# salute-developers/GigaAM

Hardware: AMD Instinct MI355X
Metric: RTFx v2_ctc batch32x20s (log-mel + encoder + greedy decode) (higher is better)
Workload: dtype f32 (GEMMs: 3-term split on fp16 MFMA, fp32 accumulate)

## Files before the change

gigaam_amd/_lib.py:

```python
from __future__ import annotations

import ctypes as C
import os
from typing import Optional

_HERE = os.path.dirname(os.path.abspath(__file__))
LIB_NAME = "libgigaam_hip.so"
LIB_PATH = os.path.join(_HERE, LIB_NAME)

SUBS_CONV2D, SUBS_CONV1D = 0, 1
ATT_ROTARY, ATT_REL_POS = 0, 1
NORM_BATCH, NORM_LAYER = 0, 1
HEAD_NONE, HEAD_CTC, HEAD_RNNT, HEAD_EMO = 0, 1, 2, 3
DTYPE_F32, DTYPE_F16, DTYPE_BF16, DTYPE_F64, DTYPE_I64 = 0, 1, 2, 3, 4
GEMM_F32, GEMM_F16X3, GEMM_F16 = 0, 1, 2
RS_U8, RS_I16, RS_I24, RS_I32, RS_F32, RS_MULAW, RS_ALAW = range(7)
RS_FORM_SINGLE, RS_FORM_TABLE, RS_FORM_ROWS = 0, 1, 2
PF_CLASSES = ["gemm", "conv2", "attn", "norm", "convmod", "stem", "frontend", "decode", "misc", "align_bt", "align_out"]


class GamConfig(C.Structure):
    _fields_ = [(n, C.c_int32) for n in (
        "sample_rate", "n_mels", "hop_length", "win_length", "n_fft", "center",
        "feat_in", "n_layers", "d_model", "subsampling", "subs_kernel_size", "subsampling_factor",
# ... 61 lines not shown
    "gam_rnnt_align": (C.c_int, [_P, _P, _P, C.c_int, C.c_int64, _P, _P, C.c_int, _P, _P, _P, _P, _P]),
    "gam_op_rnnt_align": (C.c_int, [_P, _P, _P, C.c_int, C.c_int64, _P, _P, C.c_int, _P, _P, _P, _P, _P, _P]),
    "gam_op_rnnt_lattice_align": (C.c_int, [_P, _P, _P, C.c_int, C.c_int64, C.c_int, _P, _P, C.c_int, _P, _P, _P, _P, _P]),
    "gam_set_rnnt_align_workspace": (C.c_int, [_P, C.c_int64]),
    "gam_ctc_confidence": (C.c_int, [_P, _P, _P, C.c_int, C.c_int64, _P, _P, _P, C.c_int, C.c_int, C.c_int, _P, _P, _P, _P]),
    "gam_op_ctc_confidence": (C.c_int, [_P, _P, _P, C.c_int, C.c_int64, C.c_int, _P, _P, _P, C.c_int, C.c_int, C.c_int, _P, _P, _P, _P]),
    "gam_op_ctc_confidence_long": (C.c_int, [_P, _P, C.c_int64, C.c_int, _P, _P, _P, C.c_int, C.c_int, C.c_int, C.c_int, _P, _P, _P, _P]),
    "gam_rnnt_confidence": (C.c_int, [_P, _P, _P, C.c_int, C.c_int64, _P, _P, _P, C.c_int, C.c_int, _P, _P, _P]),
    "gam_op_rnnt_confidence": (C.c_int, [_P, _P, _P, C.c_int, C.c_int64, _P, _P, _P, C.c_int, C.c_int, _P, _P, _P]),
    "gam_emo_probs": (C.c_int, [_P, _P, _P, C.c_int, C.c_int64, _P, _P]),
    "gam_rnnt_predict": (C.c_int, [_P, _P, _P, _P, C.c_int, _P, _P, _P, _P]),
    "gam_rnnt_joint": (C.c_int, [_P, _P, _P, C.c_int, C.c_int, C.c_int, _P, _P]),
    "gam_set_gemm_mode": (C.c_int, [_P, C.c_int]),
    "gam_get_gemm_mode": (C.c_int, [_P]),
    "gam_set_rnnt_cluster": (C.c_int, [_P, C.c_int]),
    "gam_get_rnnt_cluster": (C.c_int, [_P]),
    "gam_rnnt_cluster_plan_info": (C.c_int, [C.c_int] * 8 + [C.POINTER(C.c_int32)]),
    "gam_rnnt_last_decode": (C.c_int, [_P, C.POINTER(C.c_int32)]),
    "gam_debug_buffer_hash": (C.c_int, [_P, C.c_int, C.POINTER(C.c_uint64), C.POINTER(C.c_int64)]),
    "gam_range_flag": (C.c_int, [_P, C.POINTER(C.c_int), _P]),
    "gam_range_flag_fetch": (C.c_int, [_P, _P, _P]),
    "gam_op_gemm": (C.c_int, [_P, _P, _P, _P, _P, C.c_int, C.c_int, C.c_int, C.c_int, _P]),
    "gam_op_gemm_ex": (C.c_int, [_P, _P, _P, _P, _P, C.c_float, _P, C.c_int, C.c_int, C.c_int, C.c_int, _P]),
    "gam_op_attention": (C.c_int, [_P, _P, _P, _P, _P, _P, C.c_int, C.c_int, C.c_int, _P]),
    "gam_op_attention_ex": (C.c_int, [_P, _P, _P, _P, C.c_int64, _P, _P, _P, C.c_int, C.c_int, C.c_int, C.c_int, _P, _P, _P, _P]),
    "gam_op_layernorm": (C.c_int, [_P, C.POINTER(GamLnOp), _P]),
    "gam_op_convmod": (C.c_int, [_P, _P, _P, _P, _P, _P, _P, _P, _P, C.c_int, C.c_int, C.c_int, C.c_int, C.c_int, C.c_int, C.c_int, _P]),
    "gam_tune_sp": (C.c_int, [C.c_int, C.c_int, C.c_int]),
    "gam_plan_sp": (C.c_int, [C.c_int, C.c_int, C.c_int, C.c_int, C.POINTER(C.c_int), C.POINTER(C.c_int), C.POINTER(C.c_int)]),
    "gam_plan_sp_ex": (C.c_int, [C.c_int, C.c_int, C.c_int, C.c_int, C.POINTER(C.c_int), C.POINTER(C.c_int), C.POINTER(C.c_int), C.POINTER(C.c_int)]),
    "gam_tune_sp_stages": (C.c_int, [C.c_int]),
    "gam_resample_plan": (C.c_int, [C.c_int, C.c_int, C.POINTER(C.c_int), C.POINTER(C.c_int), C.POINTER(C.c_int)]),
    "gam_resample_tile": (C.c_int, [C.c_int, C.c_int, C.POINTER(C.c_int), C.POINTER(C.c_int)]),
    "gam_resample_table": (C.c_int, [C.c_int, C.c_int, _P, _P]),
    "gam_resample_out_len": (C.c_int64, [C.c_int, C.c_int, C.c_int64]),
    "gam_op_resample": (C.c_int, [_P, C.c_int, C.c_int, C.c_int, _P, C.c_int, C.c_int64, C.c_int, C.c_int, _P, _P, _P, C.c_int64, _P, _P]),
    "gam_profile_enable": (C.c_int, [_P, C.c_int]),
    "gam_profile_pause": (C.c_int, [_P, C.c_int]),
    "gam_profile_read": (C.c_int, [_P, C.c_int, C.POINTER(C.c_double), C.POINTER(C.c_int64), C.POINTER(C.c_double)]),
    "gam_profile_read_bytes": (C.c_int, [_P, C.c_int, C.POINTER(C.c_double)]),
    "gam_last_error": (C.c_char_p, [_P]),
    "gam_comm_unique_id": (C.c_int, [C.c_char_p]),
    "gam_comm_create": (C.c_int, [C.c_char_p, C.c_int, C.c_int, C.c_int, C.POINTER(_P)]),
    "gam_comm_world": (C.c_int, [_P]),
    "gam_gather_ids": (C.c_int, [_P, _P, _P, _P, _P, C.c_int, C.c_int, _P, _P, _P, _P, _P]),
    "gam_comm_last_error": (C.c_char_p, [_P]),
# ... 30 lines not shown
```

gigaam_amd/csrc/gam_api.hip:

```cpp
#include <hip/hip_runtime.h>

#include <algorithm>
#include <cmath>
#include <cstdarg>
#include <cstdio>
#include <cstring>
#include <map>
#include <string>
#include <vector>

#include "../../include/gigaam_hip.h"
#include "gam_align.h"
#include "gam_align_long.h"
#include "gam_kws.h"
#include "gam_attn.h"
#include "gam_beam.h"
#include "gam_beam_stream.h"
#include "gam_rnnt_beam.h"
#include "gam_attn16.h"
#include "gam_comm.h"
#include "gam_common.h"
#include "gam_convmod.h"
#include "gam_decode.h"
#include "gam_rnnt_align.h"
// ... 2621 lines not shown
  HIPCHK(h, hipGetLastError());
  return 0;
}

int gam_emo_probs(gam_handle* h, const float* encoded, const int32_t* enc_len, int B, int64_t Tp, float* probs,
                  void* stream) {
  if (int r = head_check(h, GAM_HEAD_EMO, nullptr)) return r;
  if (B <= 0 || Tp <= 0 || !encoded || !probs) return fail(h, -1, "bad emotion-head arguments");
  HIPCHK(h, hipSetDevice(h->device));
  hipStream_t s = (hipStream_t)stream;
  const int D = h->cfg.d_model, NC = h->cfg.num_classes;
  ProfScope ps(h, s, GAM_PF_DECODE, (double)B * D * Tp * 4.0);
  hipLaunchKernelGGL(gam_emo_head_kernel, dim3(B), dim3(256), (size_t)(D + NC) * sizeof(float), s, encoded, enc_len,
                     h->emo_w, h->emo_b, probs, D, (int)Tp, NC);
  HIPCHK(h, hipGetLastError());
  return 0;
}

int gam_op_gemm(gam_handle* h, const float* A, const float* W, const float* bias, float* C, int M, int N, int K, int act,
                void* stream) {
  return gam_op_gemm_ex(h, A, W, bias, nullptr, 1.0f, C, M, N, K, act, stream);
}

int gam_op_gemm_ex(gam_handle* h, const float* A, const float* W, const float* bias, const float* R, float alpha, float* C, int M,
                   int N, int K, int act, void* stream) {
  if (!h) return -1;
  HIPCHK(h, hipSetDevice(h->device));
  GamGemmArgs g = gemm_args(A, K, W, bias, C, N, M, N, K);
  g.R = R; g.ldr = N; g.alpha = alpha;
  hipStream_t s = (hipStream_t)stream;
  if (!split_mode(h) || K % 32 != 0 || N % 4 != 0) return gemm(h, s, g, act);
  const size_t wn = (size_t)N * K, an = (size_t)M * K;
  W16 w16;
  if (int r = ensure(h, h->op_sp, wn + 64)) return r;
  hipLaunchKernelGGL(gam_to_sp32_kernel, dim3((int)std::min<size_t>((wn / 4 + 255) / 256, 4096)), dim3(256), 0, s, W,
                     (_Float16*)h->op_sp.p, wn / 4, (const float*)nullptr, K);
  w16.sp = (_Float16*)h->op_sp.p;
  if (int r = ensure(h, h->op_rs, (size_t)M + 64)) return r;
  hipLaunchKernelGGL(gam_rowscale_kernel, dim3(gam_cdiv(M, 4)), dim3(256), 0, s, A, h->op_rs.p, M, K, (long)K);
  g.a_rs = h->op_rs.p;
  if (int r = ensure(h, h->aplanes, an + 64)) return r;
  g.Asp = (const _Float16*)h->aplanes.p;
  g.a_fmt = (h->gemm_mode == GAM_GEMM_F16 && K % 64 == 0) ? 2 : 1;
  if (g.a_fmt == 2) {
    if (int r = ensure(h, h->op_planes, wn / 2 + 64)) return r;
    w16.h16 = (_Float16*)h->op_planes.p;
    hipLaunchKernelGGL(gam_to_h16_kernel, dim3((int)std::min<size_t>((wn / 4 + 255) / 256, 4096)), dim3(256), 0, s, W, w16.h16,
                       wn / 4, (const float*)nullptr, K);
    hipLaunchKernelGGL(gam_to_h16_kernel, dim3((int)std::min<size_t>((an / 4 + 255) / 256, 8192)), dim3(256), 0, s, A,
                       (_Float16*)h->aplanes.p, an / 4, (const float*)h->op_rs.p, K);
  } else {
    hipLaunchKernelGGL(gam_to_sp32_kernel, dim3((int)std::min<size_t>((an / 4 + 255) / 256, 8192)), dim3(256), 0, s, A,
// ... 264 lines not shown
```

gigaam_amd/csrc/gam_gemm_sp.h:

```cpp
#pragma once
#include "gam_gemm.h"
#include <type_traits>
#if defined(GAM_SP_INSTRUMENT) && GAM_SP_INSTRUMENT
#include <algorithm>
#include <vector>
#endif

#ifndef GAM_SP_INSTRUMENT
#define GAM_SP_INSTRUMENT 0
#endif
#if GAM_SP_INSTRUMENT
#define GAM_SP_TL(i)                                                                  \
  if (g.tlog != nullptr && threadIdx.x == 0) {                                        \
    g.tlog[(size_t)lid * 8 + (i)] = wall_clock64();                                   \
    if ((i) == 1 || (i) == 2) g.tlog[(size_t)lid * 8 + 4 + (i)] = clock64();          \
    if ((i) == 0) g.tlog[(size_t)lid * 8 + 7] = blockIdx.x;                            \
  }
#else
#define GAM_SP_TL(i)
#endif

template <int MT, int NW, int NS = 2>
struct GamGemmSpCfg {
  static constexpr int BM = 64 * MT;
  static constexpr int BN = 64 * NW;
  static constexpr int NWAVES = 2 * NW;
  static constexpr int NT = 64 * NWAVES;
  static constexpr int A_BYTES = BM * 128;
  static constexpr int W_BYTES = BN * 128;
  static constexpr int STAGE = A_BYTES + W_BYTES;
  static constexpr int SMEM = NS * STAGE;
  static constexpr int NAI = BM / 8 / NWAVES;
  static constexpr int NWI = BN / 8 / NWAVES;
};

__device__ __forceinline__ int gam_sp_key(int row) { return ((row >> 1) & 7) ^ ((row >> 3) & 2); }

template <int ACT, int MT, int NW, int NS = 2, bool H16 = false>
__global__ __launch_bounds__(128 * NW, NW == 2 ? 2 : 1) void gam_gemm_sp_kernel(GamGemmArgs g) {
  extern __shared__ __attribute__((aligned(16))) unsigned char gam_smem_sp[];
  using Cfg = GamGemmSpCfg<MT, NW, NS>;
  constexpr int BM = Cfg::BM, BN = Cfg::BN, NAI = Cfg::NAI, NWI = Cfg::NWI, NWAVES = Cfg::NWAVES;
  typedef __attribute__((address_space(3))) void* lds_ptr_t;
  typedef const __attribute__((address_space(1))) void* glb_ptr_t;

  const int tid = threadIdx.x;
  const int lane = tid & 63;
  const int wave = __builtin_amdgcn_readfirstlane(tid >> 6);
  const int wm = wave / NW, wn = wave % NW;

  const int nbn = (g.N + BN - 1) / BN;
  const int total = gridDim.x;
  const int q8 = total >> 3, r8 = total & 7;
  const int bid = blockIdx.x;
  const int xcd = bid & 7;
  const int lid = (xcd < r8 ? xcd * (q8 + 1) : r8 * (q8 + 1) + (xcd - r8) * q8) + (bid >> 3);
  int tm = lid / nbn, tn = lid % nbn;
  if (g.skip_pad) {
    tm = bid / nbn;
    tn = bid % nbn;
  }
// ... 171 lines not shown
  for (int kt = 0; kt < nk; ++kt) {
    const int s_nxt = s_cur + 1 == NS ? 0 : s_cur + 1;
    const unsigned char* st = gam_smem_sp + s_cur * Cfg::STAGE;
    const unsigned char* sn = gam_smem_sp + s_nxt * Cfg::STAGE;
    half0(st);
    if constexpr (NS == 2) {
      __builtin_amdgcn_s_waitcnt(0x0070);
      __syncthreads();
    } else {
      asm volatile("s_waitcnt vmcnt(%0) lgkmcnt(0)\n\ts_barrier" ::"n"(VMW) : "memory");
    }
    half1(sn, s_cur);
    s_cur = s_nxt;
  }
#undef GAM_SPLD
#undef GAM_SP_RDW
#undef GAM_SP_RDA
#undef GAM_SP_MFMA
  __builtin_amdgcn_s_waitcnt(0x0070);
  GAM_SP_TL(2);

  const int mw = m0 + wm * (BM / 2), nw = n0 + wn * 64;

  const int lrow = lane & 15, lq8 = (lane >> 4) * 8;
  const float accscale = g.wscale_inv;
  f32x4 bv[2][2];
#pragma unroll
  for (int pp = 0; pp < 2; ++pp)
#pragma unroll
    for (int hf = 0; hf < 2; ++hf) {
      const int col = nw + 32 * pp + lq8 + 4 * hf;
      bv[pp][hf] = (g.bias != nullptr && col < g.N) ? *reinterpret_cast<const f32x4*>(g.bias + col) : (f32x4){0.f, 0.f, 0.f, 0.f};
    }
  const bool part = g.partial != nullptr;
  const bool need_bt = !part && (g.lens != nullptr || g.remap);
  bool r_ok[2 * MT], r_masked[2 * MT];
  long r_orow[2 * MT];
  float r_rsc[2 * MT];
  int bb = 0, tt = 0;
  if (need_bt) { bb = (mw + lrow) / g.rpb; tt = (mw + lrow) - bb * g.rpb; }
#pragma unroll
  for (int i = 0; i < 2 * MT; ++i) {
    const int row = mw + 16 * i + lrow;
    bool ok = row < g.M, masked = false;
    long orow = row;
    if (need_bt) {
      if (i > 0) {
        tt += 16;
        if (g.rpb < 16) { bb = row / g.rpb; tt = row - bb * g.rpb; }
        else if (tt >= g.rpb) { tt -= g.rpb; ++bb; }
      }
      if (ok) {
        if (g.lens != nullptr) masked = tt >= g.lens[bb] * g.fdiv;
        if (g.remap) {
          if (tt >= g.rows_valid) ok = false;
          orow = (long)bb * g.out_rpb + tt + g.out_shift;
        }
      }
    }
    r_rsc[i] = accscale * ((ok && g.a_rs != nullptr) ? g.a_rs[row] : 1.0f);
    r_ok[i] = ok; r_masked[i] = masked; r_orow[i] = orow;
  }
  if (part) {
#pragma unroll
    for (int i = 0; i < 2 * MT; ++i) {
      if (!r_ok[i]) continue;
      float* P = g.partial + ((size_t)blockIdx.y * (size_t)g.M + (size_t)(mw + 16 * i + lrow)) * (size_t)g.N;
#pragma unroll
      for (int pp = 0; pp < 2; ++pp)
#pragma unroll
        for (int hf = 0; hf < 2; ++hf) {
          const int ecol = nw + 32 * pp + lq8 + 4 * hf;
          if (ecol < g.N) *reinterpret_cast<f32x4*>(P + ecol) = acc[i][2 * pp + hf] * r_rsc[i];
        }
    }
  }
#define GAM_SP_LDR(I, D)                                                                          \
  _Pragma("unroll") for (int pp = 0; pp < 2; ++pp) _Pragma("unroll") for (int hf = 0; hf < 2; ++hf) { \
    const int col = nw + 32 * pp + lq8 + 4 * hf;                                                  \
    D[pp][hf] = (r_ok[I] && col < g.N) ? *reinterpret_cast<const f32x4*>(g.R + r_orow[I] * g.ldr + col) : (f32x4){0.f, 0.f, 0.f, 0.f}; \
  }
  f32x4 rv[2][2], rn[2][2];
  const bool resid = g.R != nullptr && !part;
  if (resid) GAM_SP_LDR(0, rv);
#pragma unroll
  for (int i = 0; i < 2 * MT; ++i) {
    if (resid && i + 1 < 2 * MT) GAM_SP_LDR(i + 1, rn);
    const bool masked = r_masked[i];
    const long orow = r_orow[i];
    const float rsc = r_rsc[i];
    if (r_ok[i] && !part) {
#pragma unroll
      for (int pp = 0; pp < 2; ++pp) {
        const int ecol = nw + 32 * pp + lq8;
        if (ecol >= g.N) continue;
        const bool both = ecol + 4 < g.N;
        f32x4 v[2];
#pragma unroll
        for (int hf = 0; hf < 2; ++hf) {
          f32x4 t = acc[i][2 * pp + hf];
          t = t * rsc + bv[pp][hf];
          if (ACT == GAM_ACT_SILU) { t.x = gam_silu(t.x); t.y = gam_silu(t.y); t.z = gam_silu(t.z); t.w = gam_silu(t.w); }
          if (ACT == GAM_ACT_RELU) { t.x = fmaxf(t.x, 0.f); t.y = fmaxf(t.y, 0.f); t.z = fmaxf(t.z, 0.f); t.w = fmaxf(t.w, 0.f); }
          if (masked) t = (f32x4){0.f, 0.f, 0.f, 0.f};
          t = t * g.alpha;
          if (resid) t += rv[pp][hf];
          if (!both && hf == 1) t = (f32x4){0.f, 0.f, 0.f, 0.f};
          v[hf] = t;
        }
        if (g.c_guard) { gam_range_note(g.range_flag, v[0].x, v[0].y, v[0].z, v[0].w); gam_range_note(g.range_flag, v[1].x, v[1].y, v[1].z, v[1].w); }
        if (g.c_split == 2) {
          _Float16* cp = reinterpret_cast<_Float16*>(g.C) + orow * g.ldc + ecol;
          const gam_half4 h0 = __builtin_convertvector(v[0], gam_half4), h1 = __builtin_convertvector(v[1], gam_half4);
          if (both) *reinterpret_cast<gam_half8*>(cp) = (gam_half8){h0[0], h0[1], h0[2], h0[3], h1[0], h1[1], h1[2], h1[3]};
          else *reinterpret_cast<gam_half4*>(cp) = h0;
        } else if (g.c_split) {
          _Float16* cp = reinterpret_cast<_Float16*>(g.C) + orow * (2 * g.ldc) + (ecol >> 5) * 64 + (ecol & 31);
          gam_half4 hi0, lo0, hi1, lo1;
          gam_split4(v[0], hi0, lo0);
          gam_split4(v[1], hi1, lo1);
          if (both) {
            *reinterpret_cast<gam_half8*>(cp) = (gam_half8){hi0[0], hi0[1], hi0[2], hi0[3], hi1[0], hi1[1], hi1[2], hi1[3]};
            *reinterpret_cast<gam_half8*>(cp + 32) = (gam_half8){lo0[0], lo0[1], lo0[2], lo0[3], lo1[0], lo1[1], lo1[2], lo1[3]};
          } else {
            *reinterpret_cast<gam_half4*>(cp) = hi0;
            *reinterpret_cast<gam_half4*>(cp + 32) = lo0;
          }
        } else {
          *reinterpret_cast<f32x4*>(g.C + orow * g.ldc + ecol) = v[0];
          if (both) *reinterpret_cast<f32x4*>(g.C + orow * g.ldc + ecol + 4) = v[1];
        }
      }
    }
    if (resid && i + 1 < 2 * MT) {
#pragma unroll
      for (int pp = 0; pp < 2; ++pp)
#pragma unroll
        for (int hf = 0; hf < 2; ++hf) rv[pp][hf] = rn[pp][hf];
    }
  }
#undef GAM_SP_LDR
#if GAM_SP_INSTRUMENT
  if (g.tlog != nullptr) { __builtin_amdgcn_s_waitcnt(0x0070); __syncthreads(); }
  GAM_SP_TL(3);
#endif
}

static inline bool gam_gemm_sp_epilogue_ok(const GamGemmArgs& a) {
  auto al16 = [](const void* p) { return (reinterpret_cast<uintptr_t>(p) & 15) == 0; };
  return a.N % 4 == 0 && a.ldc % 4 == 0 && al16(a.C) && (a.bias == nullptr || al16(a.bias)) &&
         (a.R == nullptr || (a.ldr % 4 == 0 && al16(a.R)));
}

template <int ACT, int MT, int NW, int NS = 2, bool H16 = false>
static inline void gam_launch_gemm_sp_t(const GamGemmArgs& a, int grid, hipStream_t stream) {
  static std::atomic<unsigned long long> attr_devs{0};
  constexpr int smem = GamGemmSpCfg<MT, NW, NS>::SMEM;
  static_assert(smem <= 160 * 1024, "LDS stages do not fit a CU");
  auto kern = gam_gemm_sp_kernel<ACT, MT, NW, NS, H16>;
  if (gam_set_max_lds(reinterpret_cast<const void*>(kern), smem, attr_devs) != hipSuccess) return;
  hipLaunchKernelGGL(kern, dim3(grid, a.splitk > 1 ? a.splitk : 1), dim3(128 * NW), smem, stream, a);
}

struct GamSpPlan { int mt, nw, s, ns; };
struct GamSpForce {
  std::atomic<int> mt{0}, nw{0}, s{0}, ns{0};
  GamSpForce() {
    const char* e0 = getenv("GAM_SP_MT"); const char* e1 = getenv("GAM_SP_NW"); const char* e2 = getenv("GAM_SP_SPLITK");
    const char* e3 = getenv("GAM_SP_STAGES");
    mt = e0 ? atoi(e0) : 0; nw = e1 ? atoi(e1) : 0; s = e2 ? atoi(e2) : 0; ns = e3 ? atoi(e3) : 0;
  }
};
static inline bool gam_sp_has_ns3(int mt, int nw) { return (nw == 2 && (mt == 2 || mt == 3)) || (nw == 4 && mt == 2); }
static inline GamSpForce& gam_sp_force() { static GamSpForce f; return f; }
static inline double gam_gemm_sp_model(int M, int N, int K, int a_mode, int t, int w, int S, int ncu, int ns = 2) {
  const long wgs = (long)gam_cdiv(M, 64 * t) * gam_cdiv(N, 64 * w) * S;
  const int nkt = K / 32 / S;
  double t_kt, t_fix, rounds;
  if (ns == 3) {
    if (w == 4) { t_kt = 0.953; t_fix = S > 1 ? 6.62 : 12.8; }
    else { t_kt = 0.229 * t + 0.115; t_fix = S > 1 ? 4.76 : 12.0; }
    rounds = (double)((wgs + ncu - 1) / ncu);
  } else if (w == 4) {
    t_kt = 0.335 * t + 0.425;
// ... 56 lines not shown
  int mt = a.sp_mt, nw = a.sp_nw, ns = a.sp_ns;
  if (mt < 2 || mt > 4 || (nw != 2 && nw != 4) || (nw == 2 && mt == 4)) {
    const GamSpPlan p = gam_gemm_sp_plan(a.M, a.N, a.K, a.a_mode);
    mt = p.mt; nw = p.nw; ns = p.ns;
    if (a.splitk > 1 && a.partial == nullptr) return hipErrorInvalidValue;
  }
  if (ns != 3 || !gam_sp_has_ns3(mt, nw)) ns = 2;
  if (a.splitk > 1 && (a.partial == nullptr || (a.K / 32) % a.splitk != 0)) return hipErrorInvalidValue;
  if (a.n_switch > 0 && (a.Asp2 == nullptr || a.a_mode != 0 || a.n_switch % (64 * nw) != 0)) return hipErrorInvalidValue;
  if (a.splitk <= 1) { a.splitk = 0; a.partial = nullptr; }
  const int grid = gam_cdiv(a.M, 64 * mt) * gam_cdiv(a.N, 64 * nw);
  a.ntiles = grid;
#if GAM_SP_INSTRUMENT
  static long long* tl_dev = nullptr;
  static int tl_cap = 0;
  static const bool tl_on = getenv("GAM_SP_TLOG") != nullptr;
  a.tlog = nullptr;
  if (tl_on) {
    if (grid > tl_cap) { if (tl_dev) (void)hipFree(tl_dev); (void)hipMalloc(&tl_dev, (size_t)grid * 64); tl_cap = grid; }
    (void)hipMemsetAsync(tl_dev, 0, (size_t)grid * 64, stream);
    a.tlog = tl_dev;
  }
#endif
#define GAM_LSP(ACTV)                                                            \
  if (a.h16) {           \
    if (ns == 3) {                                                               \
      if (nw == 4) gam_launch_gemm_sp_t<ACTV, 2, 4, 3, true>(a, grid, stream);   \
      else if (mt == 2) gam_launch_gemm_sp_t<ACTV, 2, 2, 3, true>(a, grid, stream); \
      else gam_launch_gemm_sp_t<ACTV, 3, 2, 3, true>(a, grid, stream);           \
    } else if (nw == 2) {                                                        \
      if (mt == 2) gam_launch_gemm_sp_t<ACTV, 2, 2, 2, true>(a, grid, stream);   \
      else gam_launch_gemm_sp_t<ACTV, 3, 2, 2, true>(a, grid, stream);           \
    } else switch (mt) {                                                         \
      case 2: gam_launch_gemm_sp_t<ACTV, 2, 4, 2, true>(a, grid, stream); break; \
      case 3: gam_launch_gemm_sp_t<ACTV, 3, 4, 2, true>(a, grid, stream); break; \
      default: gam_launch_gemm_sp_t<ACTV, 4, 4, 2, true>(a, grid, stream); break; \
    }                                                                            \
  } else if (ns == 3) {                                                          \
    if (nw == 4) gam_launch_gemm_sp_t<ACTV, 2, 4, 3>(a, grid, stream);           \
    else if (mt == 2) gam_launch_gemm_sp_t<ACTV, 2, 2, 3>(a, grid, stream);      \
    else gam_launch_gemm_sp_t<ACTV, 3, 2, 3>(a, grid, stream);                   \
  } else if (nw == 2) switch (mt) {                                              \
    case 2: gam_launch_gemm_sp_t<ACTV, 2, 2>(a, grid, stream); break;            \
    default: gam_launch_gemm_sp_t<ACTV, 3, 2>(a, grid, stream); break;           \
  } else switch (mt) {                                                           \
    case 2: gam_launch_gemm_sp_t<ACTV, 2, 4>(a, grid, stream); break;            \
    case 3: gam_launch_gemm_sp_t<ACTV, 3, 4>(a, grid, stream); break;            \
    default: gam_launch_gemm_sp_t<ACTV, 4, 4>(a, grid, stream); break;           \
  }
  switch (act) {
    case GAM_ACT_SILU: GAM_LSP(GAM_ACT_SILU); break;
    case GAM_ACT_RELU: GAM_LSP(GAM_ACT_RELU); break;
    default: GAM_LSP(GAM_ACT_NONE); break;
  }
#undef GAM_LSP
#if GAM_SP_INSTRUMENT
  if (tl_on) {
    std::vector<long long> t((size_t)grid * 8);
    (void)hipStreamSynchronize(stream);
    (void)hipMemcpy(t.data(), tl_dev, t.size() * 8, hipMemcpyDeviceToHost);
    long long t_first = t[0], t_last = 0;
    for (int i = 0; i < grid; ++i) { t_first = std::min(t_first, t[i * 8]); t_last = std::max(t_last, t[i * 8 + 3]); }
    auto stat = [&](auto f, const char* name) {
      std::vector<double> v(grid);
      for (int i = 0; i < grid; ++i) v[i] = f(i);
      std::sort(v.begin(), v.end());
      fprintf(stderr, "    %-26s min %7.2f  p50 %7.2f  p90 %7.2f  max %7.2f us\n", name, v[0], v[grid / 2], v[(size_t)(grid * 0.9)], v[grid - 1]);
    };
    fprintf(stderr, "[tlog] M=%d N=%d K=%d MT=%d NW=%d tiles=%d: first entry -> last exit %.2f us\n", a.M, a.N, a.K, mt, nw, grid, (t_last - t_first) * 0.01);
    stat([&](int i) { return (t[i * 8] - t_first) * 0.01; }, "entry after first entry");
    stat([&](int i) { return (t[i * 8 + 1] - t[i * 8]) * 0.01; }, "prologue (2 k-tiles land)");
    stat([&](int i) { return (t[i * 8 + 2] - t[i * 8 + 1]) * 0.01; }, "main loop");
    stat([&](int i) { return (t[i * 8 + 2] - t[i * 8 + 1]) * 0.01 / (a.K / 32); }, "  per k-tile");
    stat([&](int i) { return (double)(t[i * 8 + 6] - t[i * 8 + 5]) / std::max<long long>(1, t[i * 8 + 2] - t[i * 8 + 1]) * 100.0; }, "  shader MHz in loop");
    stat([&](int i) { return (t[i * 8 + 3] - t[i * 8 + 2]) * 0.01; }, "epilogue");
    stat([&](int i) { return (t_last - t[i * 8 + 3]) * 0.01; }, "idle after exit");
    double x_loop[8] = {0}; int x_n[8] = {0};
    for (int i = 0; i < grid; ++i) { const int x = (int)(t[i * 8 + 7] & 7); x_loop[x] += (t[i * 8 + 2] - t[i * 8 + 1]) * 0.01; ++x_n[x]; }
// ... 46 lines not shown
```

gigaam_amd/engine.py:

```python
from __future__ import annotations

import contextlib
import ctypes as C
import functools
import math
import os
import threading
from typing import Any, Callable, Dict, List, Mapping, Optional, Sequence, Tuple

import numpy as np
import torch
from torch import Tensor

from . import _lib
from ._lib import GamConfig, GigaAMHipError


def _get(cfg: Any, key: str, default: Any = None) -> Any:
    if cfg is None:
        return default
    if isinstance(cfg, Mapping):
        return cfg.get(key, default)
    return getattr(cfg, key, default)

# ... 1283 lines not shown
        if b != b2 or d != self.cfg.d_model or ph != self.cfg.pred_hidden:
            raise GigaAMHipError(f"joint expects [B,T,{self.cfg.d_model}] and [B,U,{self.cfg.pred_hidden}], got {tuple(enc.shape)} / {tuple(dec.shape)}")
        out = torch.empty((b, t, u, self.cfg.num_classes), dtype=torch.float32, device=self.device)
        with torch.cuda.device(self.device):
            rc = self.lib.gam_rnnt_joint(self._h, _ptr(enc), _ptr(dec), b, t, u, _ptr(out), self._stream())
        self._check(rc, "gam_rnnt_joint")
        return out

    def op_gemm(self, a: Tensor, w: Tensor, bias: Optional[Tensor] = None, act: int = 0, resid: Optional[Tensor] = None,
                alpha: float = 1.0) -> Tensor:
        a = self._dev(a, torch.float32)
        w = self._dev(w, torch.float32)
        bias = None if bias is None else self._dev(bias, torch.float32)
        resid = None if resid is None else self._dev(resid, torch.float32)
        m, k = a.shape
        n = w.shape[0]
        out = torch.empty((m, n), dtype=torch.float32, device=self.device)
        with torch.cuda.device(self.device):
            rc = self.lib.gam_op_gemm_ex(self._h, _ptr(a), _ptr(w), _ptr(bias), _ptr(resid), alpha, _ptr(out), m, n, k, act,
                                         self._stream())
        self._check(rc, "gam_op_gemm_ex")
        return out

    def op_attention(self, q: Tensor, k: Tensor, v: Tensor, lens: Optional[Tensor] = None) -> Tensor:
        q, k, v = (self._dev(t, torch.float32) for t in (q, k, v))
        b, t, d = q.shape
        lens_d = None if lens is None else self._dev(lens, torch.int32)
        out = torch.empty_like(q)
        with torch.cuda.device(self.device):
            rc = self.lib.gam_op_attention(self._h, _ptr(q), _ptr(k), _ptr(v), _ptr(out), _ptr(lens_d), b, t, d // 48, self._stream())
        self._check(rc, "gam_op_attention")
        return out

    def op_attention_ex(self, q: Tensor, k: Tensor, v: Tensor, B: int, Ta: int, Tv: int, H: int, lens: Optional[Tensor] = None,
                        cu: Optional[Tensor] = None, pbuf: Optional[Tensor] = None, pos_u: Optional[Tensor] = None,
                        pos_v: Optional[Tensor] = None) -> Tensor:
        ldq = q.stride(0)
        if not (q.is_cuda and k.is_cuda and v.is_cuda) or k.stride(0) != ldq or v.stride(0) != ldq or any(t.stride(1) != 1 for t in (q, k, v)):
            raise GigaAMHipError("op_attention_ex: q, k, v must be CUDA row views with one row stride")
        lens_d, cu_d = (None if t is None else self._dev(t, torch.int32) for t in (lens, cu))
        pbuf, pos_u, pos_v = (None if t is None else self._dev(t, torch.float32) for t in (pbuf, pos_u, pos_v))
        out = torch.full((q.shape[0], H * 48), float("nan"), dtype=torch.float32, device=self.device)
        with torch.cuda.device(self.device):
            rc = self.lib.gam_op_attention_ex(self._h, _ptr(q), _ptr(k), _ptr(v), ldq, _ptr(out), _ptr(lens_d), _ptr(cu_d), B, Ta, Tv, H,
                                              _ptr(pbuf), _ptr(pos_u), _ptr(pos_v), self._stream())
        self._check(rc, "gam_op_attention_ex")
# ... 54 lines not shown
```

include/gigaam_hip.h:

```cpp
#ifndef GIGAAM_HIP_H
#define GIGAAM_HIP_H

#include <stdint.h>

#ifdef __cplusplus
extern "C" {
#endif

#define GAM_ABI_VERSION 1

typedef struct gam_handle gam_handle;

enum { GAM_SUBS_CONV2D = 0, GAM_SUBS_CONV1D = 1 };
enum { GAM_ATT_ROTARY = 0, GAM_ATT_REL_POS = 1 };
enum { GAM_NORM_BATCH = 0, GAM_NORM_LAYER = 1 };
enum { GAM_HEAD_NONE = 0, GAM_HEAD_CTC = 1, GAM_HEAD_RNNT = 2, GAM_HEAD_EMO = 3 };
enum { GAM_DTYPE_F32 = 0, GAM_DTYPE_F16 = 1, GAM_DTYPE_BF16 = 2, GAM_DTYPE_F64 = 3, GAM_DTYPE_I64 = 4 };

typedef struct gam_config {
  int32_t sample_rate, n_mels, hop_length, win_length, n_fft, center;
  int32_t feat_in, n_layers, d_model, subsampling, subs_kernel_size, subsampling_factor;
  int32_t ff_expansion_factor, self_attention_model, n_heads, pos_emb_max_len;
  int32_t conv_norm_type, conv_kernel_size;
  int32_t head_type, num_classes, pred_hidden, pred_rnn_layers, joint_hidden;
// ... 133 lines not shown
int gam_get_rnnt_cluster(gam_handle* h);
int gam_rnnt_cluster_plan_info(int ncu, int cluster, int exclusive, int B, int H, int JH, int V, int L, int32_t* out);
int gam_rnnt_last_decode(gam_handle* h, int32_t* out);

int gam_debug_buffer_hash(gam_handle* h, int which, uint64_t* hash_out, int64_t* floats_out);

int gam_rnnt_predict(gam_handle* h, const int32_t* labels, const float* h_in, const float* c_in, int B, float* g_out,
                     float* h_out, float* c_out, void* stream);
int gam_rnnt_joint(gam_handle* h, const float* enc, const float* dec, int B, int T, int U, float* log_probs, void* stream);

int gam_emo_probs(gam_handle* h, const float* encoded, const int32_t* enc_len, int B, int64_t Tp, float* probs,
                  void* stream);

enum { GAM_GEMM_F32 = 0, GAM_GEMM_F16X3 = 1, GAM_GEMM_F16 = 2 };
int gam_set_gemm_mode(gam_handle* h, int mode);
int gam_range_flag(gam_handle* h, int* flag_host, void* stream);
int gam_range_flag_fetch(gam_handle* h, int32_t* flag_dev, void* stream);
int gam_get_gemm_mode(const gam_handle* h);

int gam_op_gemm(gam_handle* h, const float* A, const float* W, const float* bias, float* C,
                int M, int N, int K, int act, void* stream);
int gam_op_gemm_ex(gam_handle* h, const float* A, const float* W, const float* bias, const float* R, float alpha,
                   float* C, int M, int N, int K, int act, void* stream);

int gam_op_attention(gam_handle* h, const float* q, const float* k, const float* v, float* ctx,
                     const int32_t* lens, int B, int T, int H, void* stream);
int gam_op_attention_ex(gam_handle* h, const float* q, const float* k, const float* v, int64_t ldq, float* ctx,
                        const int32_t* lens, const int32_t* cu, int B, int Ta, int Tv, int H, const float* pbuf,
                        const float* pos_u, const float* pos_v, void* stream);

typedef struct gam_ln_op {
  const float* x;
  float* out1;
  float* out2;
  const float* w1;
  const float* b1;
  const float* w2;
  const float* b2;
  const float* rcos;
  const float* rsin;
  const int32_t* row_t;
  float* rs;
  const float* part;
  const float* pbias;
  const float* presid;
  float* xstore;
// ... 50 lines not shown
```

Before: 21020.

## Specialize split-precision GEMM epilogue at compile time per usage pattern

```diff
diff --git a/gigaam_amd/_lib.py b/gigaam_amd/_lib.py
--- a/gigaam_amd/_lib.py
+++ b/gigaam_amd/_lib.py
@@ -107,6 +107,7 @@
     "gam_range_flag_fetch": (C.c_int, [_P, _P, _P]),
     "gam_op_gemm": (C.c_int, [_P, _P, _P, _P, _P, C.c_int, C.c_int, C.c_int, C.c_int, _P]),
     "gam_op_gemm_ex": (C.c_int, [_P, _P, _P, _P, _P, C.c_float, _P, C.c_int, C.c_int, C.c_int, C.c_int, _P]),
+    "gam_op_gemm_fmt": (C.c_int, [_P, _P, _P, _P, _P, C.c_float, _P, C.c_int64, C.c_int, C.c_int, C.c_int, C.c_int, C.c_int, C.c_int, _P]),
     "gam_op_attention": (C.c_int, [_P, _P, _P, _P, _P, _P, C.c_int, C.c_int, C.c_int, _P]),
     "gam_op_attention_ex": (C.c_int, [_P, _P, _P, _P, C.c_int64, _P, _P, _P, C.c_int, C.c_int, C.c_int, C.c_int, _P, _P, _P, _P]),
     "gam_op_layernorm": (C.c_int, [_P, C.POINTER(GamLnOp), _P]),
diff --git a/gigaam_amd/csrc/gam_api.hip b/gigaam_amd/csrc/gam_api.hip
--- a/gigaam_amd/csrc/gam_api.hip
+++ b/gigaam_amd/csrc/gam_api.hip
@@ -2667,12 +2667,30 @@
   return gam_op_gemm_ex(h, A, W, bias, nullptr, 1.0f, C, M, N, K, act, stream);
 }
 
+static int op_gemm_impl(gam_handle* h, const float* A, const float* W, const float* bias, const float* R, float alpha, float* C, long ldc,
+                        int M, int N, int K, int act, int c_split, int c_guard, void* stream);
+
 int gam_op_gemm_ex(gam_handle* h, const float* A, const float* W, const float* bias, const float* R, float alpha, float* C, int M,
                    int N, int K, int act, void* stream) {
   if (!h) return -1;
+  return op_gemm_impl(h, A, W, bias, R, alpha, C, N, M, N, K, act, 0, 0, stream);
+}
+
+int gam_op_gemm_fmt(gam_handle* h, const float* A, const float* W, const float* bias, const float* R, float alpha, float* C, int64_t ldc,
+                    int M, int N, int K, int act, int c_split, int c_guard, void* stream) {
+  if (!h) return -1;
+  if (!split_mode(h) || K % 32 != 0 || N % 4 != 0 || ldc < N || c_split < 0 || c_split > 2 || (c_split == 1 && ldc % 32 != 0) ||
+      (c_split == 2 && !(h->gemm_mode == GAM_GEMM_F16 && K % 64 == 0)))
+    return fail(h, -1, "gam_op_gemm_fmt: format %d / pitch %ld not available for this mode and shape (N=%d K=%d)", c_split, (long)ldc, N, K);
+  return op_gemm_impl(h, A, W, bias, R, alpha, C, (long)ldc, M, N, K, act, c_split, c_guard, stream);
+}
+
+static int op_gemm_impl(gam_handle* h, const float* A, const float* W, const float* bias, const float* R, float alpha, float* C, long ldc,
+                        int M, int N, int K, int act, int c_split, int c_guard, void* stream) {
   HIPCHK(h, hipSetDevice(h->device));
-  GamGemmArgs g = gemm_args(A, K, W, bias, C, N, M, N, K);
-  g.R = R; g.ldr = N; g.alpha = alpha;
+  GamGemmArgs g = gemm_args(A, K, W, bias, C, ldc, M, N, K);
+  g.R = R; g.ldr = ldc; g.alpha = alpha;
+  g.c_split = c_split; g.c_guard = c_guard;
   hipStream_t s = (hipStream_t)stream;
   if (!split_mode(h) || K % 32 != 0 || N % 4 != 0) return gemm(h, s, g, act);
   const size_t wn = (size_t)N * K, an = (size_t)M * K;
diff --git a/gigaam_amd/csrc/gam_gemm_sp.h b/gigaam_amd/csrc/gam_gemm_sp.h
--- a/gigaam_amd/csrc/gam_gemm_sp.h
+++ b/gigaam_amd/csrc/gam_gemm_sp.h
@@ -36,7 +36,20 @@
 
 __device__ __forceinline__ int gam_sp_key(int row) { return ((row >> 1) & 7) ^ ((row >> 3) & 2); }
 
-template <int ACT, int MT, int NW, int NS = 2, bool H16 = false>
+enum : int {
+  GAM_EPI_SP32 = 1,
+  GAM_EPI_F16 = 2,
+  GAM_EPI_CFMT = 3,
+  GAM_EPI_RESID = 4,
+  GAM_EPI_ALPHA = 8,
+  GAM_EPI_ROWS = 16,
+  GAM_EPI_GUARD = 32,
+  GAM_EPI_TAIL = 64,
+  GAM_EPI_PART = 128,
+  GAM_EPI_GENERIC = 256
+};
+
+template <int ACT, int EPI, int MT, int NW, int NS = 2, bool H16 = false>
 __global__ __launch_bounds__(128 * NW, NW == 2 ? 2 : 1) void gam_gemm_sp_kernel(GamGemmArgs g) {
   extern __shared__ __attribute__((aligned(16))) unsigned char gam_smem_sp[];
   using Cfg = GamGemmSpCfg<MT, NW, NS>;
@@ -254,18 +267,35 @@
 
   const int mw = m0 + wm * (BM / 2), nw = n0 + wn * 64;
 
+  constexpr bool GEN = (EPI & GAM_EPI_GENERIC) != 0;
+  const bool part = GEN ? g.partial != nullptr : (EPI & GAM_EPI_PART) != 0;
+  const int cfmt = GEN ? g.c_split : (EPI & GAM_EPI_CFMT);
+  const bool resid = !part && (GEN ? g.R != nullptr : (EPI & GAM_EPI_RESID) != 0);
+  const bool scaled = GEN || (EPI & GAM_EPI_ALPHA) != 0;
+  const bool need_bt = !part && (GEN ? (g.lens != nullptr || g.remap) : (EPI & GAM_EPI_ROWS) != 0);
+  const bool guard = GEN ? (g.c_guard && g.range_flag != nullptr) : (EPI & GAM_EPI_GUARD) != 0;
+  const bool tail = GEN ? (g.N & 4) != 0 : (EPI & GAM_EPI_TAIL) != 0;
   const int lrow = lane & 15, lq8 = (lane >> 4) * 8;
   const float accscale = g.wscale_inv;
+  const int ecol0 = nw + lq8;
+  bool c_ok[2], c_both[2];
+#pragma unroll
+  for (int pp = 0; pp < 2; ++pp) {
+    c_ok[pp] = ecol0 + 32 * pp < g.N;
+    c_both[pp] = !tail || ecol0 + 32 * pp + 4 < g.N;
+  }
   f32x4 bv[2][2];
 #pragma unroll
   for (int pp = 0; pp < 2; ++pp)
 #pragma unroll
     for (int hf = 0; hf < 2; ++hf) {
-      const int col = nw + 32 * pp + lq8 + 4 * hf;
+      const int col = ecol0 + 32 * pp + 4 * hf;
       bv[pp][hf] = (g.bias != nullptr && col < g.N) ? *reinterpret_cast<const f32x4*>(g.bias + col) : (f32x4){0.f, 0.f, 0.f, 0.f};
     }
-  const bool part = g.partial != nullptr;
-  const bool need_bt = !part && (g.lens != nullptr || g.remap);
+  const long c_col = cfmt == 1 ? 2L * ((ecol0 >> 5) * 64 + (ecol0 & 31)) : (cfmt == 2 ? 2L * ecol0 : 4L * ecol0);
+  const long c_pitch = cfmt == 2 ? 2 * g.ldc : 4 * g.ldc;
+  const int c_step = cfmt == 2 ? 64 : 128;
+  unsigned char* const c_base = reinterpret_cast<unsigned char*>(g.C) + c_col;
   bool r_ok[2 * MT], r_masked[2 * MT];
   long r_orow[2 * MT];
   float r_rsc[2 * MT];
@@ -297,36 +327,35 @@
 #pragma unroll
     for (int i = 0; i < 2 * MT; ++i) {
       if (!r_ok[i]) continue;
-      float* P = g.partial + ((size_t)blockIdx.y * (size_t)g.M + (size_t)(mw + 16 * i + lrow)) * (size_t)g.N;
+      float* P = g.partial + ((size_t)blockIdx.y * (size_t)g.M + (size_t)(mw + 16 * i + lrow)) * (size_t)g.N + ecol0;
 #pragma unroll
       for (int pp = 0; pp < 2; ++pp)
 #pragma unroll
-        for (int hf = 0; hf < 2; ++hf) {
-          const int ecol = nw + 32 * pp + lq8 + 4 * hf;
-          if (ecol < g.N) *reinterpret_cast<f32x4*>(P + ecol) = acc[i][2 * pp + hf] * r_rsc[i];
-        }
+        for (int hf = 0; hf < 2; ++hf)
+          if (ecol0 + 32 * pp + 4 * hf < g.N) *reinterpret_cast<f32x4*>(P + 32 * pp + 4 * hf) = acc[i][2 * pp + hf] * r_rsc[i];
     }
   }
 #define GAM_SP_LDR(I, D)                                                                          \
-  _Pragma("unroll") for (int pp = 0; pp < 2; ++pp) _Pragma("unroll") for (int hf = 0; hf < 2; ++hf) { \
-    const int col = nw + 32 * pp + lq8 + 4 * hf;                                                  \
-    D[pp][hf] = (r_ok[I] && col < g.N) ? *reinterpret_cast<const f32x4*>(g.R + r_orow[I] * g.ldr + col) : (f32x4){0.f, 0.f, 0.f, 0.f}; \
+  {                                                                                               \
+    const float* rrow_ = g.R + r_orow[I] * g.ldr + ecol0;                                         \
+    _Pragma("unroll") for (int pp = 0; pp < 2; ++pp) _Pragma("unroll") for (int hf = 0; hf < 2; ++hf)  \
+      D[pp][hf] = (r_ok[I] && ecol0 + 32 * pp + 4 * hf < g.N) ? *reinterpret_cast<const f32x4*>(rrow_ + 32 * pp + 4 * hf)  \
+                                                             : (f32x4){0.f, 0.f, 0.f, 0.f};       \
   }
   f32x4 rv[2][2], rn[2][2];
-  const bool resid = g.R != nullptr && !part;
+  float gmax = 0.f;
   if (resid) GAM_SP_LDR(0, rv);
 #pragma unroll
   for (int i = 0; i < 2 * MT; ++i) {
     if (resid && i + 1 < 2 * MT) GAM_SP_LDR(i + 1, rn);
     const bool masked = r_masked[i];
-    const long orow = r_orow[i];
     const float rsc = r_rsc[i];
     if (r_ok[i] && !part) {
+      unsigned char* const crow = c_base + r_orow[i] * c_pitch;
 #pragma unroll
       for (int pp = 0; pp < 2; ++pp) {
-        const int ecol = nw + 32 * pp + lq8;
-        if (ecol >= g.N) continue;
-        const bool both = ecol + 4 < g.N;
+        if (!c_ok[pp]) continue;
+        const bool both = c_both[pp];
         f32x4 v[2];
 #pragma unroll
         for (int hf = 0; hf < 2; ++hf) {
@@ -334,33 +363,35 @@
           t = t * rsc + bv[pp][hf];
           if (ACT == GAM_ACT_SILU) { t.x = gam_silu(t.x); t.y = gam_silu(t.y); t.z = gam_silu(t.z); t.w = gam_silu(t.w); }
           if (ACT == GAM_ACT_RELU) { t.x = fmaxf(t.x, 0.f); t.y = fmaxf(t.y, 0.f); t.z = fmaxf(t.z, 0.f); t.w = fmaxf(t.w, 0.f); }
-          if (masked) t = (f32x4){0.f, 0.f, 0.f, 0.f};
-          t = t * g.alpha;
+          if (need_bt && masked) t = (f32x4){0.f, 0.f, 0.f, 0.f};
+          if (scaled) t = t * g.alpha;
           if (resid) t += rv[pp][hf];
-          if (!both && hf == 1) t = (f32x4){0.f, 0.f, 0.f, 0.f};
+          if (tail && !both && hf == 1) t = (f32x4){0.f, 0.f, 0.f, 0.f};
           v[hf] = t;
         }
-        if (g.c_guard) { gam_range_note(g.range_flag, v[0].x, v[0].y, v[0].z, v[0].w); gam_range_note(g.range_flag, v[1].x, v[1].y, v[1].z, v[1].w); }
-        if (g.c_split == 2) {
-          _Float16* cp = reinterpret_cast<_Float16*>(g.C) + orow * g.ldc + ecol;
+        if (guard) {
+          gmax = fmaxf(gmax, fmaxf(fmaxf(fabsf(v[0].x), fabsf(v[0].y)), fmaxf(fabsf(v[0].z), fabsf(v[0].w))));
+          gmax = fmaxf(gmax, fmaxf(fmaxf(fabsf(v[1].x), fabsf(v[1].y)), fmaxf(fabsf(v[1].z), fabsf(v[1].w))));
+        }
+        unsigned char* const cp = crow + pp * c_step;
+        if (cfmt == 2) {
           const gam_half4 h0 = __builtin_convertvector(v[0], gam_half4), h1 = __builtin_convertvector(v[1], gam_half4);
           if (both) *reinterpret_cast<gam_half8*>(cp) = (gam_half8){h0[0], h0[1], h0[2], h0[3], h1[0], h1[1], h1[2], h1[3]};
           else *reinterpret_cast<gam_half4*>(cp) = h0;
-        } else if (g.c_split) {
-          _Float16* cp = reinterpret_cast<_Float16*>(g.C) + orow * (2 * g.ldc) + (ecol >> 5) * 64 + (ecol & 31);
+        } else if (cfmt) {
           gam_half4 hi0, lo0, hi1, lo1;
           gam_split4(v[0], hi0, lo0);
           gam_split4(v[1], hi1, lo1);
           if (both) {
             *reinterpret_cast<gam_half8*>(cp) = (gam_half8){hi0[0], hi0[1], hi0[2], hi0[3], hi1[0], hi1[1], hi1[2], hi1[3]};
-            *reinterpret_cast<gam_half8*>(cp + 32) = (gam_half8){lo0[0], lo0[1], lo0[2], lo0[3], lo1[0], lo1[1], lo1[2], lo1[3]};
+            *reinterpret_cast<gam_half8*>(cp + 64) = (gam_half8){lo0[0], lo0[1], lo0[2], lo0[3], lo1[0], lo1[1], lo1[2], lo1[3]};
           } else {
             *reinterpret_cast<gam_half4*>(cp) = hi0;
-            *reinterpret_cast<gam_half4*>(cp + 32) = lo0;
+            *reinterpret_cast<gam_half4*>(cp + 64) = lo0;
           }
         } else {
-          *reinterpret_cast<f32x4*>(g.C + orow * g.ldc + ecol) = v[0];
-          if (both) *reinterpret_cast<f32x4*>(g.C + orow * g.ldc + ecol + 4) = v[1];
+          *reinterpret_cast<f32x4*>(cp) = v[0];
+          if (both) *reinterpret_cast<f32x4*>(cp + 16) = v[1];
         }
       }
     }
@@ -371,6 +402,7 @@
         for (int hf = 0; hf < 2; ++hf) rv[pp][hf] = rn[pp][hf];
     }
   }
+  if (guard && gmax > GAM_F16_SAFE_MAX) atomicOr(g.range_flag, 1);
 #undef GAM_SP_LDR
 #if GAM_SP_INSTRUMENT
   if (g.tlog != nullptr) { __builtin_amdgcn_s_waitcnt(0x0070); __syncthreads(); }
@@ -384,14 +416,21 @@
          (a.R == nullptr || (a.ldr % 4 == 0 && al16(a.R)));
 }
 
-template <int ACT, int MT, int NW, int NS = 2, bool H16 = false>
+template <int ACT, int EPI, int MT, int NW, int NS = 2, bool H16 = false>
 static inline void gam_launch_gemm_sp_t(const GamGemmArgs& a, int grid, hipStream_t stream) {
   static std::atomic<unsigned long long> attr_devs{0};
   constexpr int smem = GamGemmSpCfg<MT, NW, NS>::SMEM;
   static_assert(smem <= 160 * 1024, "LDS stages do not fit a CU");
-  auto kern = gam_gemm_sp_kernel<ACT, MT, NW, NS, H16>;
+  auto kern = gam_gemm_sp_kernel<ACT, EPI, MT, NW, NS, H16>;
   if (gam_set_max_lds(reinterpret_cast<const void*>(kern), smem, attr_devs) != hipSuccess) return;
   hipLaunchKernelGGL(kern, dim3(grid, a.splitk > 1 ? a.splitk : 1), dim3(128 * NW), smem, stream, a);
+}
+
+static inline int gam_sp_epi_bits(const GamGemmArgs& a) {
+  if (a.partial != nullptr) return GAM_EPI_PART;
+  return (a.c_split & GAM_EPI_CFMT) | (a.R != nullptr ? GAM_EPI_RESID : 0) | (a.alpha != 1.0f ? GAM_EPI_ALPHA : 0) |
+         ((a.lens != nullptr || a.remap) ? GAM_EPI_ROWS : 0) | ((a.c_guard && a.range_flag != nullptr) ? GAM_EPI_GUARD : 0) |
+         ((a.N & 7) == 4 ? GAM_EPI_TAIL : 0);
 }
 
 struct GamSpPlan { int mt, nw, s, ns; };
@@ -494,38 +533,58 @@
     a.tlog = tl_dev;
   }
 #endif
-#define GAM_LSP(ACTV)                                                            \
-  if (a.h16) {           \
-    if (ns == 3) {                                                               \
-      if (nw == 4) gam_launch_gemm_sp_t<ACTV, 2, 4, 3, true>(a, grid, stream);   \
-      else if (mt == 2) gam_launch_gemm_sp_t<ACTV, 2, 2, 3, true>(a, grid, stream); \
-      else gam_launch_gemm_sp_t<ACTV, 3, 2, 3, true>(a, grid, stream);           \
-    } else if (nw == 2) {                                                        \
-      if (mt == 2) gam_launch_gemm_sp_t<ACTV, 2, 2, 2, true>(a, grid, stream);   \
-      else gam_launch_gemm_sp_t<ACTV, 3, 2, 2, true>(a, grid, stream);           \
-    } else switch (mt) {                                                         \
-      case 2: gam_launch_gemm_sp_t<ACTV, 2, 4, 2, true>(a, grid, stream); break; \
-      case 3: gam_launch_gemm_sp_t<ACTV, 3, 4, 2, true>(a, grid, stream); break; \
-      default: gam_launch_gemm_sp_t<ACTV, 4, 4, 2, true>(a, grid, stream); break; \
-    }                                                                            \
-  } else if (ns == 3) {                                                          \
-    if (nw == 4) gam_launch_gemm_sp_t<ACTV, 2, 4, 3>(a, grid, stream);           \
-    else if (mt == 2) gam_launch_gemm_sp_t<ACTV, 2, 2, 3>(a, grid, stream);      \
-    else gam_launch_gemm_sp_t<ACTV, 3, 2, 3>(a, grid, stream);                   \
-  } else if (nw == 2) switch (mt) {                                              \
-    case 2: gam_launch_gemm_sp_t<ACTV, 2, 2>(a, grid, stream); break;            \
-    default: gam_launch_gemm_sp_t<ACTV, 3, 2>(a, grid, stream); break;           \
-  } else switch (mt) {                                                           \
-    case 2: gam_launch_gemm_sp_t<ACTV, 2, 4>(a, grid, stream); break;            \
-    case 3: gam_launch_gemm_sp_t<ACTV, 3, 4>(a, grid, stream); break;            \
-    default: gam_launch_gemm_sp_t<ACTV, 4, 4>(a, grid, stream); break;           \
-  }
-  switch (act) {
-    case GAM_ACT_SILU: GAM_LSP(GAM_ACT_SILU); break;
-    case GAM_ACT_RELU: GAM_LSP(GAM_ACT_RELU); break;
-    default: GAM_LSP(GAM_ACT_NONE); break;
+#define GAM_LSP(ACTV, EPIV)                                                            \
+  if (ns == 3) {                                                                       \
+    if (nw == 4) gam_launch_gemm_sp_t<ACTV, EPIV, 2, 4, 3>(a, grid, stream);           \
+    else if (mt == 2) gam_launch_gemm_sp_t<ACTV, EPIV, 2, 2, 3>(a, grid, stream);      \
+    else gam_launch_gemm_sp_t<ACTV, EPIV, 3, 2, 3>(a, grid, stream);                   \
+  } else if (nw == 2) switch (mt) {                                                    \
+    case 2: gam_launch_gemm_sp_t<ACTV, EPIV, 2, 2>(a, grid, stream); break;            \
+    default: gam_launch_gemm_sp_t<ACTV, EPIV, 3, 2>(a, grid, stream); break;           \
+  } else switch (mt) {                                                                 \
+    case 2: gam_launch_gemm_sp_t<ACTV, EPIV, 2, 4>(a, grid, stream); break;            \
+    case 3: gam_launch_gemm_sp_t<ACTV, EPIV, 3, 4>(a, grid, stream); break;            \
+    default: gam_launch_gemm_sp_t<ACTV, EPIV, 4, 4>(a, grid, stream); break;           \
+  }
+#define GAM_LSP_H16(ACTV)                                                              \
+  if (ns == 3) {                                                                       \
+    if (nw == 4) gam_launch_gemm_sp_t<ACTV, GAM_EPI_GENERIC, 2, 4, 3, true>(a, grid, stream);      \
+    else if (mt == 2) gam_launch_gemm_sp_t<ACTV, GAM_EPI_GENERIC, 2, 2, 3, true>(a, grid, stream); \
+    else gam_launch_gemm_sp_t<ACTV, GAM_EPI_GENERIC, 3, 2, 3, true>(a, grid, stream);  \
+  } else if (nw == 2) {                                                                \
+    if (mt == 2) gam_launch_gemm_sp_t<ACTV, GAM_EPI_GENERIC, 2, 2, 2, true>(a, grid, stream);      \
+    else gam_launch_gemm_sp_t<ACTV, GAM_EPI_GENERIC, 3, 2, 2, true>(a, grid, stream);  \
+  } else switch (mt) {                                                                 \
+    case 2: gam_launch_gemm_sp_t<ACTV, GAM_EPI_GENERIC, 2, 4, 2, true>(a, grid, stream); break;    \
+    case 3: gam_launch_gemm_sp_t<ACTV, GAM_EPI_GENERIC, 3, 4, 2, true>(a, grid, stream); break;    \
+    default: gam_launch_gemm_sp_t<ACTV, GAM_EPI_GENERIC, 4, 4, 2, true>(a, grid, stream); break;   \
+  }
+  const int epi = gam_sp_epi_bits(a);
+  const int act_k = epi == GAM_EPI_PART ? GAM_ACT_NONE : act;
+  enum : int { E_PLAIN = 0, E_RES = GAM_EPI_RESID, E_RESA = GAM_EPI_RESID | GAM_EPI_ALPHA, E_GRD = GAM_EPI_GUARD,
+               E_UP = GAM_EPI_SP32 | GAM_EPI_GUARD, E_STEM = GAM_EPI_SP32 | GAM_EPI_GUARD | GAM_EPI_ROWS };
+  if (a.h16) {
+    switch (act) {
+      case GAM_ACT_SILU: GAM_LSP_H16(GAM_ACT_SILU); break;
+      case GAM_ACT_RELU: GAM_LSP_H16(GAM_ACT_RELU); break;
+      default: GAM_LSP_H16(GAM_ACT_NONE); break;
+    }
+  } else if (act_k == GAM_ACT_NONE && epi == E_PLAIN) { GAM_LSP(GAM_ACT_NONE, E_PLAIN);
+  } else if (act_k == GAM_ACT_NONE && epi == E_RES) { GAM_LSP(GAM_ACT_NONE, E_RES);
+  } else if (act_k == GAM_ACT_NONE && epi == E_RESA) { GAM_LSP(GAM_ACT_NONE, E_RESA);
+  } else if (act_k == GAM_ACT_NONE && epi == E_GRD) { GAM_LSP(GAM_ACT_NONE, E_GRD);
+  } else if (act_k == GAM_ACT_SILU && epi == E_UP) { GAM_LSP(GAM_ACT_SILU, E_UP);
+  } else if (act_k == GAM_ACT_RELU && epi == E_STEM) { GAM_LSP(GAM_ACT_RELU, E_STEM);
+  } else if (epi == GAM_EPI_PART) { GAM_LSP(GAM_ACT_NONE, GAM_EPI_PART);
+  } else {
+    switch (act) {
+      case GAM_ACT_SILU: GAM_LSP(GAM_ACT_SILU, GAM_EPI_GENERIC); break;
+      case GAM_ACT_RELU: GAM_LSP(GAM_ACT_RELU, GAM_EPI_GENERIC); break;
+      default: GAM_LSP(GAM_ACT_NONE, GAM_EPI_GENERIC); break;
+    }
   }
 #undef GAM_LSP
+#undef GAM_LSP_H16
 #if GAM_SP_INSTRUMENT
   if (tl_on) {
     std::vector<long long> t((size_t)grid * 8);
diff --git a/gigaam_amd/engine.py b/gigaam_amd/engine.py
--- a/gigaam_amd/engine.py
+++ b/gigaam_amd/engine.py
@@ -1329,6 +1329,19 @@
         self._check(rc, "gam_op_gemm_ex")
         return out
 
+    def op_gemm_fmt(self, a: Tensor, w: Tensor, out: Tensor, bias: Optional[Tensor] = None, act: int = 0, resid: Optional[Tensor] = None,
+                    alpha: float = 1.0, c_split: int = 0, c_guard: bool = False) -> Tensor:
+        a = self._dev(a, torch.float32)
+        w = self._dev(w, torch.float32)
+        bias = None if bias is None else self._dev(bias, torch.float32)
+        m, k = a.shape
+        n = w.shape[0]
+        with torch.cuda.device(self.device):
+            rc = self.lib.gam_op_gemm_fmt(self._h, _ptr(a), _ptr(w), _ptr(bias), _ptr(resid), alpha, _ptr(out), out.stride(0), m, n, k, act,
+                                          int(c_split), int(bool(c_guard)), self._stream())
+        self._check(rc, "gam_op_gemm_fmt")
+        return out
+
     def op_attention(self, q: Tensor, k: Tensor, v: Tensor, lens: Optional[Tensor] = None) -> Tensor:
         q, k, v = (self._dev(t, torch.float32) for t in (q, k, v))
         b, t, d = q.shape
diff --git a/include/gigaam_hip.h b/include/gigaam_hip.h
--- a/include/gigaam_hip.h
+++ b/include/gigaam_hip.h
@@ -179,6 +179,8 @@
                 int M, int N, int K, int act, void* stream);
 int gam_op_gemm_ex(gam_handle* h, const float* A, const float* W, const float* bias, const float* R, float alpha,
                    float* C, int M, int N, int K, int act, void* stream);
+int gam_op_gemm_fmt(gam_handle* h, const float* A, const float* W, const float* bias, const float* R, float alpha,
+                    float* C, int64_t ldc, int M, int N, int K, int act, int c_split, int c_guard, void* stream);
 
 int gam_op_attention(gam_handle* h, const float* q, const float* k, const float* v, float* ctx,
                      const int32_t* lens, int B, int T, int H, void* stream);
```

Measured after the change: 21280 (median of 6 runs). 1.01x the previous value.
